# Graylab/DFMDock

Hardware: AMD Instinct MI355X
Metric: docking trajectories/sec (N_res~300+300, 40 steps) (higher is better)
Workload: dtype f16

## Files before the change

### dfmdock_amd/csrc/api_forward.hip

```cpp
#include <cstdio>
#include <cstring>
#include <vector>

#include "dfm_device.h"
#include "dfm_engine.h"

using namespace dfm;

int dfm::begin_call(dfm_complex *cx, int B, const EngineSel &sel, bool l0)
{
    int rc = ensure_workspace(cx, B, sel.bf16, l0);
    if (rc) return rc;
    cx->prof = dfm_profile{};
    cx->ev_used = 0; cx->ev_l0_used = 0;
    cx->fwd_counter = 0;
    if (l0) {
        if (!(sel.bf16 ? cx->l0_valid : cx->l0_valid32)) {
            float bms = 0.f;
            if ((rc = build_l0_table(cx, &bms, !sel.bf16)) != DFM_OK) return rc;
            cx->prof.l0_build_ms = bms;
        }
        HIPCHK(hipMemsetAsync(cx->ws.l0_miss_total, 0, sizeof(unsigned long long), cx->stream));
    }
    return DFM_OK;
// ... 205 lines not shown
        cx->prof.l0_evals += 1; cx->prof.l0_edges += (int64_t)B * N * K;
    }
    return DFM_OK;
}

static int enqueue_messages(const Fwd &f, int l, const float *h, bool lig_only)
{
    EdgeArgs e = layer_edge_args(f, l, lig_only);
    int rc = enqueue_layer_telemetry(f, l, h, e);
    if (rc) return rc;
    rc = (l == 0 && f.o.l0_table) ? enqueue_l0_table(f, e) : enqueue_message_launch(f, e);
    if (rc) return rc;
    if (e.last && f.o.bf16) HIPCHK(launch_coord_bf16(e, f.cx->stream));
    return DFM_OK;
}

static int enqueue_node_model(const Fwd &f, int l, const float *h, float *hn)
{
    dfm_complex *cx = f.cx;
    const FwdOpts &o = f.o;
    Workspace &W = cx->ws;
    hipStream_t s = cx->stream;
    const LayerDev &Lw = cx->m->layers[l];
    const int N = cx->N;
    const bool last = (l == cx->m->hp.depth - 1);
    GemmArgs g = gemm_args(h, H, 2 * H, Lw.W3, 2 * H, Lw.b3, f.M, H, W.u, H);
    g.A1 = W.agg; g.pro = 1; g.a0_period = l == 0 ? N : 0;
    const bool fused_stats = o.bf16 && gemm_rows_per_tile() == 64;
    if (fused_stats) { g.stat_part = W.gn_part; g.rows_per_graph = N; }
    HIPCHK(launch_gemm(o.bf16, g, Lw.W3_hi, Lw.W3_lo, s));
    if (!fused_stats) HIPCHK(launch_gn_stats(W.u, f.B, N, Lw.gn_ms, W.gn_shift, W.gn_den, o.bf16 ? Lw.gn_w : nullptr, o.bf16 ? Lw.gn_b : nullptr, s));
    g = gemm_args(W.u, H, H, Lw.W4, H, Lw.b4, f.M, H, hn, H);
    g.pro = 2; g.gn_shift = W.gn_shift; g.gn_den = W.gn_den; g.gn_w = Lw.gn_w; g.gn_b = Lw.gn_b; g.rows_per_graph = N;
    if (fused_stats) { g.gn_part = W.gn_part; g.gn_ms = Lw.gn_ms; }
    if (o.bf16 && !last && f.tile_tasks) g.zbuf = W.agg;
    g.epi = 1; g.R = h; g.r_period = l == 0 ? N : 0;
    HIPCHK(launch_gemm(o.bf16, g, Lw.W4_hi, Lw.W4_lo, s));
    return DFM_OK;
}

static int enqueue_next_ab(const Fwd &f, int l, const float *h)
{
    dfm_complex *cx = f.cx;
    const FwdOpts &o = f.o;
    Workspace &W = cx->ws;
    const LayerDev &Ln = cx->m->layers[l];
    const float *bias = cx->homomer ? (o.bf16 ? Ln.bias_ab_h_s : Ln.bias_ab_h) : (o.bf16 ? Ln.bias_ab_s : Ln.bias_ab);
    GemmArgs g = gemm_args(h, H, H, Ln.Wab, H, bias, f.M, 2 * H, W.A, H);
    g.epi = 2; g.C2 = o.bf16 ? nullptr : W.Bm; g.C2b = W.Bmb;
    if (o.bf16 && !o.f16) g.Cb = reinterpret_cast<uint16_t *>(W.A);
    HIPCHK(launch_gemm(o.bf16, g, Ln.Wab_hi, Ln.Wab_lo, cx->stream));
    return DFM_OK;
}

static int enqueue_pair_head(const Fwd &f, int q, int mode)
{
    dfm_complex *cx = f.cx;
    const dfm_model *m = cx->m;
    Workspace &W = cx->ws;
    hipStream_t s = cx->stream;
    const int R = cx->R;
    const PairHeadDev &Ph = m->pair[q];
    HIPCHK(project_ab(cx, f.B, Ph.wab, Ph.wab_hi, Ph.wab_lo, f.o.bf16));
    PairArgs a;
    std::memset(&a, 0, sizeof(a));
    a.P = W.A; a.Q = W.Bm; a.ca4 = W.ca4; a.B = f.B; a.R = R; a.L = cx->L; a.w_d = Ph.w_d; a.ln_w = Ph.ln_w; a.ln_b = Ph.ln_b;
    a.w3 = Ph.w3; a.mode = mode; a.cut_off = m->hp.cut_off; a.fpart = W.fpart;
    a.spart = mode == 1 ? W.en_part : W.cpart; a.clash_part = W.clash_part;
    if (f.o.bf16) {
        a.S = W.pair_s; a.Rp = (R + 31) / 32 * 32;
        HIPCHK(launch_pair_head_m(a, s));
        HIPCHK(launch_pair_finish_s(a, 4 * ((R + 63) / 64), m->hp.agg_mean ? 1.0f / (float)R : 1.0f, W.fvec, W.conf, s));
        return DFM_OK;
    }
    HIPCHK(launch_pair_head(a, s));
    return DFM_OK;
}

static int enqueue_pair_heads(const Fwd &f)
{
    dfm_complex *cx = f.cx;
    const dfm_model *m = cx->m;
    Workspace &W = cx->ws;
// ... 13 lines not shown
{
    dfm_complex *cx = f.cx;
    const dfm_model *m = cx->m;
    Workspace &W = cx->ws;
    hipStream_t s = cx->stream;
    GemmArgs g = gemm_args(W.h, H, H, m->heads.en_wa, 2 * H, nullptr, f.M, H, W.A, H);
    HIPCHK(launch_gemm_f32(g, s));
    g.W = m->heads.en_wb; g.C = W.Bm;
    HIPCHK(launch_gemm_f32(g, s));
    HIPCHK(launch_energy_pairs(W.A, W.Bm, W.ca4, f.B, cx->R, cx->L, m->hp.cut_off, &m->heads, 1, W.en_part, W.clash_part, s));
    return DFM_OK;
}

int dfm::enqueue_forward(dfm_complex *cx, int B, const FwdOpts &o)
{
    const dfm_model *m = cx->m;
    Workspace &W = cx->ws;
    hipStream_t s = cx->stream;
    const int depth = m->hp.depth;
    const Fwd f{cx, o, B, B * cx->N, m->hp.family == 1, o.bf16 && edge_msg_tile_tasks(B, cx->N, cx->K)};
    int rc = enqueue_graph(f, cx->fwd_counter++);
    if (rc) return rc;
    const float *h = cx->h0;
    float *hn = W.h, *hspare = W.h2;
    for (int l = 0; l < depth; ++l) {
        const bool last = (l == depth - 1);
        const bool lig_only = last && !f.pair_family && !o.need_node_out;
        if ((rc = enqueue_messages(f, l, h, lig_only)) != DFM_OK) return rc;
        if (lig_only) break;
        if ((rc = enqueue_node_model(f, l, h, hn)) != DFM_OK) return rc;
        { float *done = hn; hn = (l == 0) ? hspare : const_cast<float *>(h); h = done; }
        if (l == 0 && o.h_first_out)
            HIPCHK(hipMemcpyAsync(o.h_first_out, h, (size_t)f.M * H * sizeof(float), hipMemcpyDeviceToDevice, s));
        if (!last && (rc = enqueue_next_ab(f, l + 1, h)) != DFM_OK) return rc;
    }
    if (o.range && (o.need_node_out || f.pair_family)) HIPCHK(launch_absmax(h, (long long)f.M * H, o.range + depth * 8, s));
    if (h != W.h && (o.need_node_out || f.pair_family))
        HIPCHK(hipMemcpyAsync(W.h, h, (size_t)f.M * H * sizeof(float), hipMemcpyDeviceToDevice, s));
    if (f.pair_family) return enqueue_pair_heads(f);
    if (o.want_energy) return enqueue_energy_head(f);
    return DFM_OK;
}

int dfm::finish_profile(dfm_complex *cx)
{
    float ms = 0.f;
    HIPCHK(hipEventElapsedTime(&ms, cx->ev_total[0], cx->ev_total[1]));
    cx->prof.total_ms = ms;
    for (size_t i = 0; i + 1 < cx->ev_used; i += 2) {
        HIPCHK(hipEventElapsedTime(&ms, cx->ev[i], cx->ev[i + 1]));
        cx->prof.edge_kernel_ms += ms;
        if (i / 2 < cx->ev_lig.size() && cx->ev_lig[i / 2]) cx->prof.edge_lig_ms += ms;
    }
    for (size_t i = 0; i + 2 < cx->ev_l0_used; i += 3) {
        HIPCHK(hipEventElapsedTime(&ms, cx->ev_l0[i], cx->ev_l0[i + 1]));
        cx->prof.l0_rows_ms += ms;
        HIPCHK(hipEventElapsedTime(&ms, cx->ev_l0[i + 1], cx->ev_l0[i + 2]));
        cx->prof.l0_gather_ms += ms;
    }
    if (cx->prof.l0_evals > 0 && cx->ws.l0_miss_total) {
        unsigned long long tot = 0;
        HIPCHK(hipMemcpyAsync(&tot, cx->ws.l0_miss_total, sizeof(tot), hipMemcpyDeviceToHost, cx->stream));
        HIPCHK(hipStreamSynchronize(cx->stream));
        cx->prof.l0_miss_rows = (int64_t)tot;
    }
#if !defined(DFM_EDGE_STAMP) && !defined(DFM_EDGE_TRACE)
    if (cx->stamp_dev && cx->ev_used) {
// ... 40 lines not shown
```

### dfmdock_amd/csrc/dfm_internal.h

```cpp
#pragma once

#include <hip/hip_runtime.h>
#include <cstdlib>
#include <stdint.h>

#include <atomic>

#include "../../include/dfmdock_amd.h"
#include "dfm_schedule.h"
#include "dfm_walkgrid.h"

namespace dfm {

constexpr int H = 256;
constexpr int HE = 128;
constexpr int HI = 128;
constexpr int NTAB = 166;
constexpr int KPAD = 64;
constexpr int MAX_NODES = 4096;
constexpr float SILU_S = -1.44269504088896340736f;

__host__ __device__ inline uint32_t pack_code(int d, int om, int th, int ph, int rp)
{
    return (uint32_t)d | ((uint32_t)om << 6) | ((uint32_t)th << 11) | ((uint32_t)ph << 16) | ((uint32_t)rp << 20);
// ... 69 lines not shown
    if (e != hipSuccess) return e;
    if (dev < 0 || dev >= MAX_DEVICES) return hipErrorInvalidDevice;
    if (done[dev].load(std::memory_order_acquire)) return hipSuccess;
    e = hipFuncSetAttribute(fn, hipFuncAttributeMaxDynamicSharedMemorySize, bytes);
    if (e == hipSuccess) done[dev].store(true, std::memory_order_release);
    return e;
}

struct GemmArgs {
    const float *A0;
    const float *A1;
    int lda;
    int K;
    const float *W;
    int ldw;
    const float *bias;
    int M, Nout;
    int pro;
    const float *gn_shift;
    const float *gn_den;
    const float *gn_w, *gn_b;
    int rows_per_graph;
    int epi;
    const float *R;
    float *C;
    int ldc;
    float *C2;
    uint16_t *C2b;
    uint16_t *Cb;
    float *stat_part;
    const float *gn_part, *gn_ms;
    float *zbuf;
    int a0_period, r_period;
};
hipError_t launch_gemm_f32(const GemmArgs &a, hipStream_t s);
hipError_t launch_gemm_split(const GemmArgs &a, const uint16_t *Whi, const uint16_t *Wlo, hipStream_t s);
int gemm_rows_per_tile();

inline unsigned token_lds()
{
    static const unsigned v = [] { const char *e = getenv("DFM_TOKEN_LDS"); return e ? (unsigned)atoi(e) : 64u; }();
    return v;
}

hipError_t launch_prep_pose(const float *rec_pos, const float *lig_cur, int B, int R, int L, int all_atoms, float4 *n4,
                            float4 *ca4, float4 *cb4, hipStream_t s);
hipError_t launch_knn_sample(const float4 *ca4, int B, int N, int knn, int nsamp, uint64_t seed, uint32_t stream_id,
                             int32_t *edges, const uint32_t *ctl, hipStream_t s);
struct L0Classify {
    const uint2 *code0;
    uint32_t *src;
    uint4 *rows;
    uint32_t *counter;
};
hipError_t launch_edge_feat(const float4 *n4, const float4 *ca4, const float4 *cb4, const int32_t *edges, int B,
                            int N, int R, int K, float mask_dist, uint32_t *codes, float *radial, const L0Classify &cls,
                            uint32_t *eval_ctr , hipStream_t s);
hipError_t launch_l0_pairs(const float4 *n4, const float4 *ca4, const float4 *cb4, int R, int L, float mask_dist, uint2 *code0,
                           uint4 *rows, hipStream_t s);

constexpr int TASK_CTR_WGS = 1024;
struct EdgeArgs {
    const float *A;
    const float *Bm;
    const uint16_t *Bmb;
    const uint16_t *Ah;
    int64_t ab_bstride;
    const int32_t *edges;
    const uint32_t *codes;
    const float *radial;
// ... 316 lines not shown
```

### dfmdock_amd/csrc/kernels_dense.hip

```cpp
#include <cstdlib>
#include "dfm_device.h"
#include "dfm_internal.h"

namespace dfm {

typedef float f32x16 __attribute__((ext_vector_type(16)));

constexpr int BM = 128, BN = 128, BK = 16, LDT = BM + 1;

__global__ __launch_bounds__(256) void k_gemm_f32(GemmArgs a)
{
    __shared__ float As[BK * LDT];
    __shared__ float Ws[BK * LDT];
    const int tid = threadIdx.x, lane = tid & 63, wave = tid >> 6;
    const int wm = wave >> 1, wn = wave & 1;
    const int row0 = blockIdx.x * BM, col0 = blockIdx.y * BN;

    f32x16 acc[2][2];
#pragma unroll
    for (int i = 0; i < 2; ++i)
#pragma unroll
        for (int j = 0; j < 2; ++j)
#pragma unroll
            for (int r = 0; r < 16; ++r) acc[i][j][r] = 0.f;

    const int lr = tid >> 2;
    const int lk = (tid & 3) * 4;
    const int halfK = a.K >> 1;

    for (int k0 = 0; k0 < a.K; k0 += BK) {
#pragma unroll
        for (int rr = 0; rr < 2; ++rr) {
            const int r = lr + rr * 64;
            const int grow = row0 + r;
            const int grow_a = a.a0_period ? grow % a.a0_period : grow;
// ... 215 lines not shown
#pragma unroll
        for (int u = 0; u < GN_CH; ++u) {
            const int t = t0 + u;
            if (t < tpt) {
                const double nt = (double)(N - t * 32 < 32 ? N - t * 32 : 32), m = (double)v[u].x, w = nt * m;
                S1 += w; S2 += w * m; SM += (double)v[u].y;
            }
        }
    }
    const double mean = S1 / N;
    const double M2 = SM + (S2 - mean * S1);
    const float sft = (float)mean * mean_scale[c];
    const double dm = mean - (double)sft;
    double var = M2 / N + dm * dm;
    var = var > 0 ? var : 0;
    const float dn = sqrtf((float)var + 1e-5f);
    if (fold_w) {
        const float sc = fold_w[c] / dn;
        o_den = sc;
        o_shift = fold_b[c] - sc * sft;
    } else {
        o_shift = sft;
        o_den = dn;
    }
}

typedef __bf16 bf16x8 __attribute__((ext_vector_type(8)));
union FragB { uint4 u; bf16x8 b; };
constexpr int SK = 32, SLD = 40;

struct GemmSplitArgs {
    GemmArgs g;
    const uint16_t *Whi, *Wlo;
};

__device__ inline uint32_t pack2(__bf16 a, __bf16 b)
{
    union { __bf16 h[2]; uint32_t u; } v;
    v.h[0] = a; v.h[1] = b;
    return v.u;
}

template <int HALF, int NJ, int QT = 0, int RING = QT> __global__ __launch_bounds__(256, RING ? 1 : 3) void k_gemm_split(GemmSplitArgs sa)
{
    static_assert(!QT || NJ == 1, "quarter tiles: one 32-column tile per wave");
    static_assert(!RING || NJ == 1, "the register ring is sized for the 64 x 128 and 64 x 64 shapes");
    static_assert(!QT || RING, "quarter tiles always run the ring");
    constexpr int MI = QT ? 1 : 2;
    constexpr int SM = 64, SN = QT ? 64 : NJ * 128;
    const GemmArgs &a = sa.g;
#ifdef DFM_GEMM_STAMP
    const unsigned long long g_entry = __builtin_amdgcn_s_memtime(), g_rt0 = __builtin_amdgcn_s_memrealtime();
#endif
    constexpr int LDS_BUF = (2 * SM + 2 * SN) * SLD;
    constexpr int LDS_OPER = (RING ? 2 : 1) * LDS_BUF, LDS_EPI = 4 * 32 * 72 * 2;
    constexpr int LDS_U16 = LDS_OPER > LDS_EPI ? LDS_OPER : LDS_EPI;
    __shared__ __attribute__((aligned(16))) uint16_t lds[LDS_U16];
    uint16_t *Ah = lds, *Al = lds + SM * SLD, *Wh = lds + 2 * SM * SLD, *Wl = lds + (2 * SM + SN) * SLD;
    const int tid = threadIdx.x, lane = tid & 63, wave = tid >> 6;
    const int wm = QT ? wave >> 1 : 0, wn = QT ? wave & 1 : wave, l31 = lane & 31;
    __shared__ __attribute__((aligned(16))) float gn_s[2 * H];
    const int vb = blockIdx.x;
    int bx = vb, by = blockIdx.y;
    if (NJ == 2 && gridDim.y == 1 && a.Nout == 2 * SN) {
        const int g16 = bx >> 4, j = bx & 15;
        bx = g16 * 8 + (j & 7); by = j >> 3;
        if (bx * SM >= a.M) return;
    }
    int row0 = bx * SM, row_end = a.M, gn_tb = 0;
    const int col0 = by * SN;
    if (a.stat_part || a.pro == 2) {
        const int tpt = (a.rows_per_graph + SM - 1) / SM, tb = bx / tpt;
        row0 = tb * a.rows_per_graph + (bx - tb * tpt) * SM;
        row_end = (tb + 1) * a.rows_per_graph;
        gn_tb = tb;
    }
    if (a.zbuf) {
        const int zr = tid >> 2;
        if (row0 + zr < row_end) {
            float4 *z = reinterpret_cast<float4 *>(a.zbuf + (size_t)(row0 + zr) * H + col0 + (tid & 3) * (SN / 4));
#pragma unroll
            for (int q = 0; q < SN / 16; ++q) z[q] = make_float4(0.f, 0.f, 0.f, 0.f);
        }
    }
    constexpr int LPR = SN * 4 / 128, NTOUCH = QT ? (SM * LPR + 255) / 256 : 0;
    float touch[NTOUCH + 1];
#pragma unroll
    for (int q = 0; q < NTOUCH; ++q) {
        touch[q] = 0.f;
        const int t = tid + q * 256, row = row0 + t / LPR;
        if (a.epi == 1 && t < SM * LPR && row < row_end) {
            const int rrow = a.r_period ? row % a.r_period : row;
            touch[q] = a.R[(size_t)rrow * a.ldc + col0 + (t % LPR) * 32];
        }
    }
    f32x16 acc[MI][NJ];
#pragma unroll
    for (int i = 0; i < MI; ++i)
#pragma unroll
        for (int j = 0; j < NJ; ++j)
#pragma unroll
            for (int r = 0; r < 16; ++r) acc[i][j][r] = 0.f;

    const int ar = tid >> 2, kg = (tid & 3) * 8;
    const int halfK = a.K >> 1;
    const bool rv0 = row0 + ar < row_end;
    const size_t gr0 = (size_t)(rv0 ? row0 + ar : 0);
    const size_t gr0a = a.a0_period ? gr0 % (size_t)a.a0_period : gr0;

    float4 xa0, xa1;
    uint4 wh0, wh1, wh2, wh3, wl0, wl1, wl2, wl3;
    const int wcol = QT ? (tid & 63) : (NJ == 2 ? tid : (tid & 127));
    const int wkq = QT ? (tid >> 7) * 2 : 0;
    const uint16_t *wsrc = QT ? (((tid >> 6) & 1) ? sa.Wlo : sa.Whi) : ((NJ == 2 || tid < 128) ? sa.Whi : sa.Wlo);
#define GEMM_SPLIT_FETCH(K0)                                                                                          \
    {                                                                                                                 \
        const int k_ = (K0) + kg;                                                                                     \
        const bool second_ = a.pro == 1 && k_ >= halfK;                                                               \
        const float *s0_ = second_ ? a.A1 + (k_ - halfK) + gr0 * a.lda : a.A0 + k_ + gr0a * a.lda;                    \
        xa0 = *reinterpret_cast<const float4 *>(s0_); xa1 = *reinterpret_cast<const float4 *>(s0_ + 4);              \
        const size_t wbase_ = ((size_t)((K0) / SK) * 4 * a.Nout + col0 + wcol) * 8;                                   \
        const size_t wq_ = (size_t)a.Nout * 8;                                                                        \
        const uint16_t *ph_ = wsrc + wbase_ + wkq * wq_, *pl_ = sa.Wlo + wbase_;                                      \
        wh0 = *reinterpret_cast<const uint4 *>(ph_); wh1 = *reinterpret_cast<const uint4 *>(ph_ + wq_);               \
        if constexpr (!QT) {                                                                                          \
            wh2 = *reinterpret_cast<const uint4 *>(ph_ + 2 * wq_); wh3 = *reinterpret_cast<const uint4 *>(ph_ + 3 * wq_); \
        }                                                                                                             \
        if constexpr (NJ == 2) {                                                                                      \
            wl0 = *reinterpret_cast<const uint4 *>(pl_); wl1 = *reinterpret_cast<const uint4 *>(pl_ + wq_);               \
            wl2 = *reinterpret_cast<const uint4 *>(pl_ + 2 * wq_); wl3 = *reinterpret_cast<const uint4 *>(pl_ + 3 * wq_); \
        }                                                                                                             \
    }
    auto stage_row = [&](const float4 &v0, const float4 &v1, bool , int k, int row, int boff = 0) {
        float x[8] = {v0.x, v0.y, v0.z, v0.w, v1.x, v1.y, v1.z, v1.w};
        if (a.pro == 2) {
            const float4 c0 = *reinterpret_cast<const float4 *>(&gn_s[k]), c1 = *reinterpret_cast<const float4 *>(&gn_s[k + 4]);
            const float4 h0 = *reinterpret_cast<const float4 *>(&gn_s[H + k]), h1 = *reinterpret_cast<const float4 *>(&gn_s[H + k + 4]);
            const float cc[8] = {c0.x, c0.y, c0.z, c0.w, c1.x, c1.y, c1.z, c1.w};
            const float hh[8] = {h0.x, h0.y, h0.z, h0.w, h1.x, h1.y, h1.z, h1.w};
#pragma unroll
            for (int e = 0; e < 8; ++e) {
                const float y = fmaf(x[e], cc[e], hh[e]);
                x[e] = y * __builtin_amdgcn_rcpf(1.0f + __expf(-y));
            }
        }
        uint32_t hi[4], lo[4];
#pragma unroll
        for (int e = 0; e < 4; ++e) {
            const float x0 = x[2 * e], x1 = x[2 * e + 1];
            const __bf16 b0 = (__bf16)x0, b1 = (__bf16)x1;
            hi[e] = pack2(b0, b1);
            lo[e] = pack2((__bf16)(x0 - (float)b0), (__bf16)(x1 - (float)b1));
        }
// ... 12 lines not shown
#endif
    float bias_r[NJ];
#pragma unroll
    for (int j = 0; j < NJ; ++j) bias_r[j] = a.bias ? a.bias[col0 + (wn * NJ + j) * 32 + l31] : 0.f;
    constexpr int QD = RING ? 4 : 1, RW = QT ? 2 : 4;
    float4 rxa0[QD], rxa1[QD];
    uint4 rw[QD][RW];
    GEMM_SPLIT_FETCH(0)
#define RING_TAKE(d) { rxa0[d] = xa0; rxa1[d] = xa1; rw[d][0] = wh0; rw[d][1] = wh1; if constexpr (!QT) { rw[d][2] = wh2; rw[d][3] = wh3; } }
#define RING_WSTORE(d, nb) { _Pragma("unroll") for (int q_ = 0; q_ < RW; ++q_) *reinterpret_cast<uint4 *>(&wdst[(nb) + wu + 8 * q_]) = rw[d][q_]; }
    if constexpr (RING) {
        RING_TAKE(0)
#pragma unroll
        for (int d = 1; d < QD; ++d) {
            GEMM_SPLIT_FETCH((d * SK < a.K ? d : 0) * SK)
            RING_TAKE(d)
        }
    }
    if (a.pro == 2) {
        if (a.gn_part) {
            float sc, sh;
            gn_finish_col(a.gn_part, gn_tb, a.rows_per_graph, tid, a.gn_ms, a.gn_w, a.gn_b, sc, sh);
            gn_s[tid] = sc; gn_s[H + tid] = sh;
        } else if (tid < 128) {
            const float *src = (tid < 64 ? a.gn_den : a.gn_shift) + (size_t)gn_tb * H + (tid & 63) * 4;
            *reinterpret_cast<float4 *>(&gn_s[(tid < 64 ? 0 : H) + (tid & 63) * 4]) = *reinterpret_cast<const float4 *>(src);
        }
        __syncthreads();
    }
    auto mfma_stage = [&](int boff = 0) {
#pragma unroll
        for (int ks = 0; ks < SK; ks += 16) {
            const int ko = ks + (lane >> 5) * 8;
            FragB ah[MI], al[MI];
#pragma unroll
            for (int i = 0; i < MI; ++i) {
                const int r = (wm * MI + i) * 32 + l31;
                ah[i].u = *reinterpret_cast<const uint4 *>(&Ah[boff + r * SLD + ko]);
                al[i].u = *reinterpret_cast<const uint4 *>(&Al[boff + r * SLD + ko]);
            }
#pragma unroll
            for (int j = 0; j < NJ; ++j) {
                const int c = (wn * NJ + j) * 32 + l31;
                FragB wh, wl;
                wh.u = *reinterpret_cast<const uint4 *>(&Wh[boff + c * SLD + ko]);
                wl.u = *reinterpret_cast<const uint4 *>(&Wl[boff + c * SLD + ko]);
#pragma unroll
                for (int i = 0; i < MI; ++i) {
                    acc[i][j] = __builtin_amdgcn_mfma_f32_32x32x16_bf16(al[i].b, wh.b, acc[i][j], 0, 0, 0);
                    acc[i][j] = __builtin_amdgcn_mfma_f32_32x32x16_bf16(ah[i].b, wl.b, acc[i][j], 0, 0, 0);
                    acc[i][j] = __builtin_amdgcn_mfma_f32_32x32x16_bf16(ah[i].b, wh.b, acc[i][j], 0, 0, 0);
                }
            }
        }
    };
    if constexpr (RING) {
        const int S = a.K / SK;
        stage_row(rxa0[0], rxa1[0], rv0, kg, ar, 0);
        RING_WSTORE(0, 0)
        {
            GEMM_SPLIT_FETCH((QD < S ? QD : S - 1) * SK)
            RING_TAKE(0)
        }
        __syncthreads();
        GSTAMP(1)
        for (int k0 = 0; k0 < S; k0 += QD) {
#pragma unroll
            for (int d = 0; d < QD; ++d) {
                const int k = k0 + d;
                const int dn = (d + 1) % QD, nb = ((d + 1) & 1) * LDS_BUF;
                const int kn = k + 1 < S ? k + 1 : S - 1, kf = k + 1 + QD < S ? k + 1 + QD : S - 1;
                mfma_stage((d & 1) * LDS_BUF);
                GSTAMP(0)
                stage_row(rxa0[dn], rxa1[dn], rv0, kn * SK + kg, ar, nb);
                RING_WSTORE(dn, nb)
                {
                    GEMM_SPLIT_FETCH(kf * SK)
                    RING_TAKE(dn)
                }
                GSTAMP(1)
                __syncthreads();
                GSTAMP(2)
            }
        }
    } else {
        for (int k0 = 0; k0 < a.K; k0 += SK) {
            if (k0) __syncthreads();
            GSTAMP(0)
            stage_row(xa0, xa1, rv0, k0 + kg, ar);
            *reinterpret_cast<uint4 *>(&wdst[wu]) = wh0; *reinterpret_cast<uint4 *>(&wdst[wu + 8]) = wh1;
            if constexpr (!QT) { *reinterpret_cast<uint4 *>(&wdst[wu + 16]) = wh2; *reinterpret_cast<uint4 *>(&wdst[wu + 24]) = wh3; }
            if constexpr (NJ == 2) {
                *reinterpret_cast<uint4 *>(&Wl[wu]) = wl0; *reinterpret_cast<uint4 *>(&Wl[wu + 8]) = wl1;
                *reinterpret_cast<uint4 *>(&Wl[wu + 16]) = wl2; *reinterpret_cast<uint4 *>(&Wl[wu + 24]) = wl3;
            }
            GSTAMP(1)
            __syncthreads();
            GSTAMP(2)
            if (k0 + SK < a.K) GEMM_SPLIT_FETCH(k0 + SK)
            mfma_stage();
        }
    }
#pragma unroll
    for (int q = 0; q < NTOUCH; ++q) asm volatile("" :: "v"(touch[q]));
    GSTAMP(0)
    __syncthreads();
    constexpr int ELD = 72;
    float *est = reinterpret_cast<float *>(lds) + wave * (32 * ELD);
    const int er = lane >> 4, ec = (lane & 15) * 4;
    float st_s[MI][4], st_q[MI][4], st_p[MI][4], st_n[MI];
#pragma unroll
    for (int i = 0; i < MI; ++i) {
        st_n[i] = 0.f;
#pragma unroll
        for (int e = 0; e < 4; ++e) { st_s[i][e] = 0.f; st_q[i][e] = 0.f; st_p[i][e] = 0.f; }
    }
#pragma unroll
    for (int i = 0; i < MI; ++i)
#pragma unroll
        for (int jp = 0; jp < (NJ + 1) / 2; ++jp) {
            float4 res[8];
            if (a.epi == 1) {
#pragma unroll
                for (int q = 0; q < 8; ++q) {
                    const size_t row = (size_t)row0 + (wm * MI + i) * 32 + q * 4 + er;
                    const size_t rrow = a.r_period ? row % (size_t)a.r_period : row;
                    const int col = col0 + (wn * NJ + jp * 2) * 32 + ec;
                    res[q] = (row < (size_t)row_end && ec < NJ * 32) ? *reinterpret_cast<const float4 *>(a.R + rrow * a.ldc + col) : make_float4(0.f, 0.f, 0.f, 0.f);
                }
            }
#pragma unroll
            for (int jj = 0; jj < (NJ < 2 ? NJ : 2); ++jj) {
                const int j = jp * 2 + jj;
                const float bias = bias_r[j];
#pragma unroll
                for (int r = 0; r < 16; ++r)
                    est[((r & 3) + 8 * (r >> 2) + 4 * (lane >> 5)) * ELD + jj * 32 + l31] = acc[i][j][r] + bias;
            }
            asm volatile("s_waitcnt lgkmcnt(0)" ::: "memory");
            if constexpr (HALF) {
                uint16_t *half_out = col0 < H ? a.Cb : a.C2b;
                const int er8 = lane >> 3, ec8 = (lane & 7) * 8;
#pragma unroll
                for (int q = 0; q < 4; ++q) {
                    const int lr = q * 8 + er8;
                    const float4 v0 = *reinterpret_cast<const float4 *>(est + lr * ELD + ec8);
                    const float4 v1 = *reinterpret_cast<const float4 *>(est + lr * ELD + ec8 + 4);
                    const size_t row = (size_t)row0 + (wm * MI + i) * 32 + lr;
                    const int col = (col0 < H ? col0 : col0 - H) + (wn * NJ + jp * 2) * 32 + ec8;
                    if (row >= (size_t)row_end || ec8 >= NJ * 32) continue;
                    uint4 o;
// ... 18 lines not shown
                        st_q[i][0] += d0 * d0; st_q[i][1] += d1 * d1; st_q[i][2] += d2 * d2; st_q[i][3] += d3 * d3;
                        st_n[i] += 1.f;
                    }
                }
                if (a.epi == 1) {
                    const float4 rr = res[q];
                    *reinterpret_cast<float4 *>(a.C + row * a.ldc + col) = make_float4(rr.x + v.x, rr.y + v.y, rr.z + v.z, rr.w + v.w);
                } else if (a.epi == 2) {
                    if (col0 < H) {
                        if (a.Cb) {
                            uint2 o;
                            o.x = pack_h2_sat(v.x, v.y);
                            o.y = pack_h2_sat(v.z, v.w);
                            *reinterpret_cast<uint2 *>(a.Cb + row * H + col) = o;
                        } else *reinterpret_cast<float4 *>(a.C + row * H + col) = v;
                    } else {
                        if (a.C2) *reinterpret_cast<float4 *>(a.C2 + row * H + (col - H)) = v;
                        if (a.C2b) {
                            uint2 o;
                            o.x = pack_h2_sat(v.x, v.y);
                            o.y = pack_h2_sat(v.z, v.w);
                            *reinterpret_cast<uint2 *>(a.C2b + row * H + (col - H)) = o;
                        }
                    }
                } else {
                    *reinterpret_cast<float4 *>(a.C + row * a.ldc + col) = v;
                }
            }
            }
            asm volatile("s_waitcnt lgkmcnt(0)" ::: "memory");
        }
    if (a.stat_part) {
#pragma clang fp contract(off)
        const int tpt64 = (a.rows_per_graph + 63) / 64, tpt32 = (a.rows_per_graph + 31) / 32;
#pragma unroll
        for (int i = 0; i < MI; ++i) {
            const int sub = (vb % tpt64) * 2 + wm * MI + i;
            float *sp = a.stat_part + ((size_t)(vb / tpt64) * tpt32 + sub) * (H * 2);
            const float inv_n = st_n[i] > 0.f ? 1.0f / st_n[i] : 0.f;
            float nl[2], fl[2];
            {
                float ne = st_n[i];
#pragma unroll
                for (int lv = 0; lv < 2; ++lv) {
                    const float n2 = __shfl_xor(ne, 16 << lv, 64), nt = ne + n2;
                    nl[lv] = ne;
                    fl[lv] = nt > 0.f ? n2 / nt : 0.f;
                    ne = nt;
                }
            }
#pragma unroll
            for (int e = 0; e < 4; ++e) {
                float mean = st_p[i][e] + st_s[i][e] * inv_n, M2 = st_q[i][e] - st_s[i][e] * st_s[i][e] * inv_n;
#pragma unroll
                for (int lv = 0; lv < 2; ++lv) {
                    const float mean2 = __shfl_xor(mean, 16 << lv, 64), M22 = __shfl_xor(M2, 16 << lv, 64);
                    const float d = mean2 - mean, f = fl[lv];
                    mean += d * f;
                    M2 += M22 + d * d * nl[lv] * f;
                }
                if (er == 0 && ec < NJ * 32 && sub < tpt32) {
                    const int c = col0 + wn * (NJ * 32) + ec + e;
                    sp[c * 2] = mean;
                    sp[c * 2 + 1] = M2;
                }
            }
        }
    }
#ifdef DFM_GEMM_STAMP
    GSTAMP(3)
    if (vb == (gridDim.x > 2048 ? 7 * 8 + 1536 : 3) && blockIdx.y == 0 && tid == 0 && a.C) {
        const unsigned long long g_rt1 = __builtin_amdgcn_s_memrealtime();
        printf("gemm stamp K=%d Nout=%d pro=%d epi=%d stats=%d gn=%d: entry->loop %llu  mfma+barrier %llu  fetch-wait+stage %llu  barrier2 %llu  epilogue %llu  total %llu shader cycles in %llu ticks of 100 MHz = %llu MHz\n",
               a.K, a.Nout, a.pro, a.epi, a.stat_part ? 1 : 0, a.gn_part ? 1 : 0, g_first - g_entry, gs[0], gs[1], gs[2], gs[3], gprev - g_entry, g_rt1 - g_rt0,
               (g_rt1 > g_rt0) ? 100ull * (gprev - g_entry) / (g_rt1 - g_rt0) : 0ull);
    }
#endif
}
#undef GEMM_SPLIT_FETCH

int gemm_rows_per_tile() { return 64; }

hipError_t launch_gemm_split(const GemmArgs &a, const uint16_t *Whi, const uint16_t *Wlo, hipStream_t s)
{
    constexpr int SN = 256;
    if (a.K % SK != 0 || a.Nout % SN != 0 || (a.pro == 1 && (a.K / 2) % SK != 0) || a.lda % 4 != 0 || a.ldc % 4 != 0)
        return hipErrorInvalidValue;
    GemmSplitArgs sa;
    sa.g = a; sa.Whi = Whi; sa.Wlo = Wlo;
    if (a.stat_part && (a.Nout != SN || a.rows_per_graph < 1 || a.M % a.rows_per_graph != 0)) return hipErrorInvalidValue;
    if (a.pro == 2 && (a.rows_per_graph < 1 || a.M % a.rows_per_graph != 0)) return hipErrorInvalidValue;
    if (a.zbuf && a.Nout != SN) return hipErrorInvalidValue;
    const int row_tiles = (a.stat_part || a.pro == 2) ? (a.M / a.rows_per_graph) * ((a.rows_per_graph + 63) / 64) : (a.M + 63) / 64;
    static const int narrow_env = [] {
        const char *e = getenv("DFM_GEMM_NARROW_MAXWG");
        return e ? atoi(e) : -1;
    }();
    const int narrow_max = narrow_env >= 0 ? narrow_env : 2 * device_cus();
    const bool narrow = (long long)row_tiles * (a.Nout / SN) < narrow_max;
    const bool half = a.epi == 2 && a.Cb && a.C2b && !a.C2;
    if (narrow) {
        static const int quarter_env = [] {
            const char *e = getenv("DFM_GEMM_QUARTER_MAXWG");
            return e ? atoi(e) : -1;
        }();
        const int quarter_max = quarter_env >= 0 ? quarter_env : device_cus() / 2;
        if ((long long)row_tiles * (a.Nout / 128) < quarter_max && (a.K / 32) % 4 == 0) {
            const dim3 grid(row_tiles, a.Nout / 64);
            if (half) hipLaunchKernelGGL((k_gemm_split<1, 1, 1>), grid, dim3(256), 0, s, sa);
            else hipLaunchKernelGGL((k_gemm_split<0, 1, 1>), grid, dim3(256), 0, s, sa);
            return hipGetLastError();
        }
        const dim3 grid(row_tiles, a.Nout / 128);
        if (half) hipLaunchKernelGGL((k_gemm_split<1, 1>), grid, dim3(256), 0, s, sa);
        else hipLaunchKernelGGL((k_gemm_split<0, 1>), grid, dim3(256), 0, s, sa);
        return hipGetLastError();
    }
    dim3 grid;
    if (a.stat_part || a.pro == 2) grid = dim3(row_tiles, a.Nout / SN);
    else if (a.Nout == 2 * SN) grid = dim3((((a.M + 63) / 64 + 7) / 8) * 16, 1);
    else grid = dim3((a.M + 63) / 64, a.Nout / SN);
    if (half) hipLaunchKernelGGL((k_gemm_split<1, 2>), grid, dim3(256), 0, s, sa);
    else hipLaunchKernelGGL((k_gemm_split<0, 2>), grid, dim3(256), 0, s, sa);
    return hipGetLastError();
}

__global__ __launch_bounds__(256) void k_gn_stats(const float *__restrict__ u, int N, const float *__restrict__ mean_scale,
                                                  float *__restrict__ shift, float *__restrict__ den,
                                                  const float *__restrict__ fold_w, const float *__restrict__ fold_b)
{
    __shared__ double red[16][64];
// ... 13 lines not shown
        __syncthreads();
    };
    double s[4] = {0, 0, 0, 0};
    for (int n = rl; n < N; n += 16) {
        const float4 v = *reinterpret_cast<const float4 *>(U + (size_t)n * H);
        s[0] += v.x; s[1] += v.y; s[2] += v.z; s[3] += v.w;
    }
    reduce_rows(s);
    if (threadIdx.x < 64) sh_shift[threadIdx.x] = (float)(red[0][threadIdx.x] / N) * mean_scale[c0 + threadIdx.x];
    __syncthreads();
    const float4 sft = *reinterpret_cast<const float4 *>(&sh_shift[cq * 4]);
    double v2[4] = {0, 0, 0, 0};
    for (int n = rl; n < N; n += 16) {
        const float4 v = *reinterpret_cast<const float4 *>(U + (size_t)n * H);
        const float o0 = v.x - sft.x, o1 = v.y - sft.y, o2 = v.z - sft.z, o3 = v.w - sft.w;
        v2[0] += (double)o0 * o0; v2[1] += (double)o1 * o1; v2[2] += (double)o2 * o2; v2[3] += (double)o3 * o3;
    }
    reduce_rows(v2);
    if (threadIdx.x < 64) {
        const int c = c0 + threadIdx.x;
        const float var = (float)(red[0][threadIdx.x] / N);
        const float dn = sqrtf(var + 1e-5f), sf = sh_shift[threadIdx.x];
        if (fold_w) {
            const float sc = fold_w[c] / dn;
            den[(size_t)b * H + c] = sc;
            shift[(size_t)b * H + c] = fold_b[c] - sc * sf;
        } else {
            shift[(size_t)b * H + c] = sf;
            den[(size_t)b * H + c] = dn;
        }
    }
}

hipError_t launch_gn_stats(const float *u, int B, int N, const float *mean_scale, float *shift, float *den,
                           const float *fold_w, const float *fold_b, hipStream_t s)
{
    hipLaunchKernelGGL(k_gn_stats, dim3(B, 4), dim3(256), 0, s, u, N, mean_scale, shift, den, fold_w, fold_b);
    return hipGetLastError();
}

}
```

Baseline: 456.4.

## Skip dead GEMM work: lean tail tiles, receptor-only rows, one-time GN finish

Adds a lean mode, on by default, with three parts. In the node-model GEMMs, partial tail tiles with fewer than 32 live rows run a single-row-block variant in which only two waves stage A, so MFMA and loads on padding rows are skipped. In the last layer's A/B projection for ligand-only output, tiles covering only receptor rows in the first half of the columns exit early. GroupNorm statistics are finished once by a small separate kernel instead of redundantly inside every W4 GEMM tile, at the cost of an extra launch. The tile-to-trajectory mapping is also reordered so full tiles come first, which adds complexity in the stat_part indexing.

```diff
diff --git a/dfmdock_amd/csrc/api_forward.hip b/dfmdock_amd/csrc/api_forward.hip
--- a/dfmdock_amd/csrc/api_forward.hip
+++ b/dfmdock_amd/csrc/api_forward.hip
@@ -261,14 +261,16 @@
     if (!fused_stats) HIPCHK(launch_gn_stats(W.u, f.B, N, Lw.gn_ms, W.gn_shift, W.gn_den, o.bf16 ? Lw.gn_w : nullptr, o.bf16 ? Lw.gn_b : nullptr, s));
     g = gemm_args(W.u, H, H, Lw.W4, H, Lw.b4, f.M, H, hn, H);
     g.pro = 2; g.gn_shift = W.gn_shift; g.gn_den = W.gn_den; g.gn_w = Lw.gn_w; g.gn_b = Lw.gn_b; g.rows_per_graph = N;
-    if (fused_stats) { g.gn_part = W.gn_part; g.gn_ms = Lw.gn_ms; }
+    const bool finish_once = fused_stats && gemm_finish_once(f.B, N);
+    if (finish_once) HIPCHK(launch_gn_finish(W.gn_part, f.B, N, Lw.gn_ms, Lw.gn_w, Lw.gn_b, W.gn_den, W.gn_shift, s));
+    else if (fused_stats) { g.gn_part = W.gn_part; g.gn_ms = Lw.gn_ms; }
     if (o.bf16 && !last && f.tile_tasks) g.zbuf = W.agg;
     g.epi = 1; g.R = h; g.r_period = l == 0 ? N : 0;
     HIPCHK(launch_gemm(o.bf16, g, Lw.W4_hi, Lw.W4_lo, s));
     return DFM_OK;
 }
 
-static int enqueue_next_ab(const Fwd &f, int l, const float *h)
+static int enqueue_next_ab(const Fwd &f, int l, const float *h, bool lig_only)
 {
     dfm_complex *cx = f.cx;
     const FwdOpts &o = f.o;
@@ -278,6 +280,7 @@
     GemmArgs g = gemm_args(h, H, H, Ln.Wab, H, bias, f.M, 2 * H, W.A, H);
     g.epi = 2; g.C2 = o.bf16 ? nullptr : W.Bm; g.C2b = W.Bmb;
     if (o.bf16 && !o.f16) g.Cb = reinterpret_cast<uint16_t *>(W.A);
+    if (lig_only && o.bf16 && !o.range && !o.sat) { g.lig_N = cx->N; g.lig_R = cx->R; }
     HIPCHK(launch_gemm(o.bf16, g, Ln.Wab_hi, Ln.Wab_lo, cx->stream));
     return DFM_OK;
 }
@@ -357,7 +360,8 @@
         { float *done = hn; hn = (l == 0) ? hspare : const_cast<float *>(h); h = done; }
         if (l == 0 && o.h_first_out)
             HIPCHK(hipMemcpyAsync(o.h_first_out, h, (size_t)f.M * H * sizeof(float), hipMemcpyDeviceToDevice, s));
-        if (!last && (rc = enqueue_next_ab(f, l + 1, h)) != DFM_OK) return rc;
+        const bool next_lig_only = (l + 1 == depth - 1) && !f.pair_family && !o.need_node_out;
+        if (!last && (rc = enqueue_next_ab(f, l + 1, h, next_lig_only)) != DFM_OK) return rc;
     }
     if (o.range && (o.need_node_out || f.pair_family)) HIPCHK(launch_absmax(h, (long long)f.M * H, o.range + depth * 8, s));
     if (h != W.h && (o.need_node_out || f.pair_family))
diff --git a/dfmdock_amd/csrc/dfm_gemm_map.h b/dfmdock_amd/csrc/dfm_gemm_map.h
--- /dev/null
+++ b/dfmdock_amd/csrc/dfm_gemm_map.h
@@ -0,0 +1,36 @@
+#pragma once
+
+#if defined(__HIPCC__) || defined(__CUDACC__)
+#define DFM_MAP_FN __host__ __device__ inline
+#else
+#define DFM_MAP_FN inline
+#endif
+
+namespace dfm {
+
+struct GemmTile {
+    int traj;
+    int tile;
+};
+
+DFM_MAP_FN GemmTile gemm_aligned_tile(int vb, int rows_per_graph, int M, int lean)
+{
+    const int tpt = (rows_per_graph + 63) / 64, full = rows_per_graph / 64;
+    GemmTile t;
+    if (!lean || full == tpt || full == 0) {
+        t.traj = vb / tpt; t.tile = vb - t.traj * tpt;
+        return t;
+    }
+    const int n_full = (M / rows_per_graph) * full;
+    if (vb < n_full) { t.traj = vb / full; t.tile = vb - t.traj * full; }
+    else { t.traj = vb - n_full; t.tile = full; }
+    return t;
+}
+
+DFM_MAP_FN bool gemm_rows_receptor_only(int row0, int row_end, int N, int R)
+{
+    const int p = row0 % N;
+    return p < R && row_end <= row0 - p + R;
+}
+
+}
diff --git a/dfmdock_amd/csrc/dfm_internal.h b/dfmdock_amd/csrc/dfm_internal.h
--- a/dfmdock_amd/csrc/dfm_internal.h
+++ b/dfmdock_amd/csrc/dfm_internal.h
@@ -125,10 +125,15 @@
     const float *gn_part, *gn_ms;
     float *zbuf;
     int a0_period, r_period;
+    int lig_N, lig_R;
 };
 hipError_t launch_gemm_f32(const GemmArgs &a, hipStream_t s);
 hipError_t launch_gemm_split(const GemmArgs &a, const uint16_t *Whi, const uint16_t *Wlo, hipStream_t s);
 int gemm_rows_per_tile();
+bool gemm_lean();
+bool gemm_finish_once(int B, int N);
+hipError_t launch_gn_finish(const float *part, int B, int N, const float *mean_scale, const float *fold_w, const float *fold_b,
+                            float *den, float *shift, hipStream_t s);
 
 inline unsigned token_lds()
 {
diff --git a/dfmdock_amd/csrc/kernels_dense.hip b/dfmdock_amd/csrc/kernels_dense.hip
--- a/dfmdock_amd/csrc/kernels_dense.hip
+++ b/dfmdock_amd/csrc/kernels_dense.hip
@@ -1,6 +1,8 @@
 #include <cstdlib>
+#include <type_traits>
 #include "dfm_device.h"
 #include "dfm_internal.h"
+#include "dfm_gemm_map.h"
 
 namespace dfm {
 
@@ -282,6 +284,7 @@
 struct GemmSplitArgs {
     GemmArgs g;
     const uint16_t *Whi, *Wlo;
+    int lean;
 };
 
 __device__ inline uint32_t pack2(__bf16 a, __bf16 b)
@@ -291,48 +294,22 @@
     return v.u;
 }
 
-template <int HALF, int NJ, int QT = 0, int RING = QT> __global__ __launch_bounds__(256, RING ? 1 : 3) void k_gemm_split(GemmSplitArgs sa)
-{
-    static_assert(!QT || NJ == 1, "quarter tiles: one 32-column tile per wave");
-    static_assert(!RING || NJ == 1, "the register ring is sized for the 64 x 128 and 64 x 64 shapes");
-    static_assert(!QT || RING, "quarter tiles always run the ring");
-    constexpr int MI = QT ? 1 : 2;
+template <int HALF, int NJ, int QT, int RING, bool DEAD>
+__device__ __forceinline__ void gemm_split_tile(const GemmSplitArgs &sa, uint16_t *lds, float *gn_s, int row0, int row_end, int col0,
+                                                int gn_tb, int tile_in)
+{
+    constexpr int MI = QT ? 1 : 2, ML = DEAD ? 1 : MI;
     constexpr int SM = 64, SN = QT ? 64 : NJ * 128;
+    constexpr int LDS_BUF = (2 * SM + 2 * SN) * SLD;
     const GemmArgs &a = sa.g;
 #ifdef DFM_GEMM_STAMP
     const unsigned long long g_entry = __builtin_amdgcn_s_memtime(), g_rt0 = __builtin_amdgcn_s_memrealtime();
+    const int vb = blockIdx.x;
 #endif
-    constexpr int LDS_BUF = (2 * SM + 2 * SN) * SLD;
-    constexpr int LDS_OPER = (RING ? 2 : 1) * LDS_BUF, LDS_EPI = 4 * 32 * 72 * 2;
-    constexpr int LDS_U16 = LDS_OPER > LDS_EPI ? LDS_OPER : LDS_EPI;
-    __shared__ __attribute__((aligned(16))) uint16_t lds[LDS_U16];
     uint16_t *Ah = lds, *Al = lds + SM * SLD, *Wh = lds + 2 * SM * SLD, *Wl = lds + (2 * SM + SN) * SLD;
     const int tid = threadIdx.x, lane = tid & 63, wave = tid >> 6;
     const int wm = QT ? wave >> 1 : 0, wn = QT ? wave & 1 : wave, l31 = lane & 31;
-    __shared__ __attribute__((aligned(16))) float gn_s[2 * H];
-    const int vb = blockIdx.x;
-    int bx = vb, by = blockIdx.y;
-    if (NJ == 2 && gridDim.y == 1 && a.Nout == 2 * SN) {
-        const int g16 = bx >> 4, j = bx & 15;
-        bx = g16 * 8 + (j & 7); by = j >> 3;
-        if (bx * SM >= a.M) return;
-    }
-    int row0 = bx * SM, row_end = a.M, gn_tb = 0;
-    const int col0 = by * SN;
-    if (a.stat_part || a.pro == 2) {
-        const int tpt = (a.rows_per_graph + SM - 1) / SM, tb = bx / tpt;
-        row0 = tb * a.rows_per_graph + (bx - tb * tpt) * SM;
-        row_end = (tb + 1) * a.rows_per_graph;
-        gn_tb = tb;
-    }
-    if (a.zbuf) {
-        const int zr = tid >> 2;
-        if (row0 + zr < row_end) {
-            float4 *z = reinterpret_cast<float4 *>(a.zbuf + (size_t)(row0 + zr) * H + col0 + (tid & 3) * (SN / 4));
-#pragma unroll
-            for (int q = 0; q < SN / 16; ++q) z[q] = make_float4(0.f, 0.f, 0.f, 0.f);
-        }
-    }
+    const int wave_u = __builtin_amdgcn_readfirstlane(wave);
     constexpr int LPR = SN * 4 / 128, NTOUCH = QT ? (SM * LPR + 255) / 256 : 0;
     float touch[NTOUCH + 1];
 #pragma unroll
@@ -344,9 +321,9 @@
             touch[q] = a.R[(size_t)rrow * a.ldc + col0 + (t % LPR) * 32];
         }
     }
-    f32x16 acc[MI][NJ];
-#pragma unroll
-    for (int i = 0; i < MI; ++i)
+    f32x16 acc[ML][NJ];
+#pragma unroll
+    for (int i = 0; i < ML; ++i)
 #pragma unroll
         for (int j = 0; j < NJ; ++j)
 #pragma unroll
@@ -363,12 +340,16 @@
     const int wcol = QT ? (tid & 63) : (NJ == 2 ? tid : (tid & 127));
     const int wkq = QT ? (tid >> 7) * 2 : 0;
     const uint16_t *wsrc = QT ? (((tid >> 6) & 1) ? sa.Wlo : sa.Whi) : ((NJ == 2 || tid < 128) ? sa.Whi : sa.Wlo);
-#define GEMM_SPLIT_FETCH(K0)                                                                                          \
+#define GEMM_SPLIT_FETCH_A(K0)                                                                                        \
     {                                                                                                                 \
         const int k_ = (K0) + kg;                                                                                     \
         const bool second_ = a.pro == 1 && k_ >= halfK;                                                               \
         const float *s0_ = second_ ? a.A1 + (k_ - halfK) + gr0 * a.lda : a.A0 + k_ + gr0a * a.lda;                    \
         xa0 = *reinterpret_cast<const float4 *>(s0_); xa1 = *reinterpret_cast<const float4 *>(s0_ + 4);              \
+    }
+#define GEMM_SPLIT_FETCH(K0) GEMM_SPLIT_FETCH_A(K0) GEMM_SPLIT_FETCH_W(K0)
+#define GEMM_SPLIT_FETCH_W(K0)                                                                                        \
+    {                                                                                                                 \
         const size_t wbase_ = ((size_t)((K0) / SK) * 4 * a.Nout + col0 + wcol) * 8;                                   \
         const size_t wq_ = (size_t)a.Nout * 8;                                                                        \
         const uint16_t *ph_ = wsrc + wbase_ + wkq * wq_, *pl_ = sa.Wlo + wbase_;                                      \
@@ -447,9 +428,9 @@
 #pragma unroll
         for (int ks = 0; ks < SK; ks += 16) {
             const int ko = ks + (lane >> 5) * 8;
-            FragB ah[MI], al[MI];
-#pragma unroll
-            for (int i = 0; i < MI; ++i) {
+            FragB ah[ML], al[ML];
+#pragma unroll
+            for (int i = 0; i < ML; ++i) {
                 const int r = (wm * MI + i) * 32 + l31;
                 ah[i].u = *reinterpret_cast<const uint4 *>(&Ah[boff + r * SLD + ko]);
                 al[i].u = *reinterpret_cast<const uint4 *>(&Al[boff + r * SLD + ko]);
@@ -461,7 +442,7 @@
                 wh.u = *reinterpret_cast<const uint4 *>(&Wh[boff + c * SLD + ko]);
                 wl.u = *reinterpret_cast<const uint4 *>(&Wl[boff + c * SLD + ko]);
 #pragma unroll
-                for (int i = 0; i < MI; ++i) {
+                for (int i = 0; i < ML; ++i) {
                     acc[i][j] = __builtin_amdgcn_mfma_f32_32x32x16_bf16(al[i].b, wh.b, acc[i][j], 0, 0, 0);
                     acc[i][j] = __builtin_amdgcn_mfma_f32_32x32x16_bf16(ah[i].b, wl.b, acc[i][j], 0, 0, 0);
                     acc[i][j] = __builtin_amdgcn_mfma_f32_32x32x16_bf16(ah[i].b, wh.b, acc[i][j], 0, 0, 0);
@@ -499,10 +480,11 @@
             }
         }
     } else {
+        const bool stager = wave_u < 2;
         for (int k0 = 0; k0 < a.K; k0 += SK) {
             if (k0) __syncthreads();
             GSTAMP(0)
-            stage_row(xa0, xa1, rv0, k0 + kg, ar);
+            if (!DEAD || stager) stage_row(xa0, xa1, rv0, k0 + kg, ar);
             *reinterpret_cast<uint4 *>(&wdst[wu]) = wh0; *reinterpret_cast<uint4 *>(&wdst[wu + 8]) = wh1;
             if constexpr (!QT) { *reinterpret_cast<uint4 *>(&wdst[wu + 16]) = wh2; *reinterpret_cast<uint4 *>(&wdst[wu + 24]) = wh3; }
             if constexpr (NJ == 2) {
@@ -512,7 +494,10 @@
             GSTAMP(1)
             __syncthreads();
             GSTAMP(2)
-            if (k0 + SK < a.K) GEMM_SPLIT_FETCH(k0 + SK)
+            if (k0 + SK < a.K) {
+                if (!DEAD || stager) GEMM_SPLIT_FETCH_A(k0 + SK)
+                GEMM_SPLIT_FETCH_W(k0 + SK)
+            }
             mfma_stage();
         }
     }
@@ -523,15 +508,15 @@
     constexpr int ELD = 72;
     float *est = reinterpret_cast<float *>(lds) + wave * (32 * ELD);
     const int er = lane >> 4, ec = (lane & 15) * 4;
-    float st_s[MI][4], st_q[MI][4], st_p[MI][4], st_n[MI];
-#pragma unroll
-    for (int i = 0; i < MI; ++i) {
+    float st_s[ML][4], st_q[ML][4], st_p[ML][4], st_n[ML];
+#pragma unroll
+    for (int i = 0; i < ML; ++i) {
         st_n[i] = 0.f;
 #pragma unroll
         for (int e = 0; e < 4; ++e) { st_s[i][e] = 0.f; st_q[i][e] = 0.f; st_p[i][e] = 0.f; }
     }
 #pragma unroll
-    for (int i = 0; i < MI; ++i)
+    for (int i = 0; i < ML; ++i)
 #pragma unroll
         for (int jp = 0; jp < (NJ + 1) / 2; ++jp) {
             float4 res[8];
@@ -616,11 +601,11 @@
         }
     if (a.stat_part) {
 #pragma clang fp contract(off)
-        const int tpt64 = (a.rows_per_graph + 63) / 64, tpt32 = (a.rows_per_graph + 31) / 32;
-#pragma unroll
-        for (int i = 0; i < MI; ++i) {
-            const int sub = (vb % tpt64) * 2 + wm * MI + i;
-            float *sp = a.stat_part + ((size_t)(vb / tpt64) * tpt32 + sub) * (H * 2);
+        const int tpt32 = (a.rows_per_graph + 31) / 32;
+#pragma unroll
+        for (int i = 0; i < ML; ++i) {
+            const int sub = tile_in * 2 + wm * MI + i;
+            float *sp = a.stat_part + ((size_t)gn_tb * tpt32 + sub) * (H * 2);
             const float inv_n = st_n[i] > 0.f ? 1.0f / st_n[i] : 0.f;
             float nl[2], fl[2];
             {
@@ -662,8 +647,70 @@
 #endif
 }
 #undef GEMM_SPLIT_FETCH
+#undef GEMM_SPLIT_FETCH_A
+#undef GEMM_SPLIT_FETCH_W
+
+template <int HALF, int NJ, int QT = 0, int RING = QT> __global__ __launch_bounds__(256, RING ? 1 : 3) void k_gemm_split(GemmSplitArgs sa)
+{
+    static_assert(!QT || NJ == 1, "quarter tiles: one 32-column tile per wave");
+    static_assert(!RING || NJ == 1, "the register ring is sized for the 64 x 128 and 64 x 64 shapes");
+    static_assert(!QT || RING, "quarter tiles always run the ring");
+    constexpr int SM = 64, SN = QT ? 64 : NJ * 128;
+    const GemmArgs &a = sa.g;
+    constexpr int LDS_BUF = (2 * SM + 2 * SN) * SLD;
+    constexpr int LDS_OPER = (RING ? 2 : 1) * LDS_BUF, LDS_EPI = 4 * 32 * 72 * 2;
+    constexpr int LDS_U16 = LDS_OPER > LDS_EPI ? LDS_OPER : LDS_EPI;
+    __shared__ __attribute__((aligned(16))) uint16_t lds[LDS_U16];
+    __shared__ __attribute__((aligned(16))) float gn_s[2 * H];
+    const int vb = blockIdx.x;
+    int bx = vb, by = blockIdx.y;
+    if (NJ == 2 && gridDim.y == 1 && a.Nout == 2 * SN) {
+        const int g16 = bx >> 4, j = bx & 15;
+        bx = g16 * 8 + (j & 7); by = j >> 3;
+        if (bx * SM >= a.M) return;
+    }
+    int row0 = bx * SM, row_end = a.M, gn_tb = 0, tile_in = 0;
+    const int col0 = by * SN;
+    if (a.lig_N && col0 < H && gemm_rows_receptor_only(row0, row0 + SM < a.M ? row0 + SM : a.M, a.lig_N, a.lig_R)) return;
+    if (a.stat_part || a.pro == 2) {
+        const GemmTile gt = gemm_aligned_tile(bx, a.rows_per_graph, a.M, NJ == 2 ? sa.lean : 0);
+        row0 = gt.traj * a.rows_per_graph + gt.tile * SM;
+        row_end = (gt.traj + 1) * a.rows_per_graph;
+        gn_tb = gt.traj; tile_in = gt.tile;
+    }
+    const bool dead1 = NJ == 2 && sa.lean && row0 + 32 >= row_end;
+    const int tid = threadIdx.x;
+    if (a.zbuf) {
+        const int zr = tid >> 2;
+        if (row0 + zr < row_end) {
+            float4 *z = reinterpret_cast<float4 *>(a.zbuf + (size_t)(row0 + zr) * H + col0 + (tid & 3) * (SN / 4));
+#pragma unroll
+            for (int q = 0; q < SN / 16; ++q) z[q] = make_float4(0.f, 0.f, 0.f, 0.f);
+        }
+    }
+    if constexpr (NJ == 2 && !HALF) {
+        if (dead1) gemm_split_tile<HALF, NJ, QT, RING, true>(sa, lds, gn_s, row0, row_end, col0, gn_tb, tile_in);
+        else gemm_split_tile<HALF, NJ, QT, RING, false>(sa, lds, gn_s, row0, row_end, col0, gn_tb, tile_in);
+    } else {
+        gemm_split_tile<HALF, NJ, QT, RING, false>(sa, lds, gn_s, row0, row_end, col0, gn_tb, tile_in);
+    }
+}
 
 int gemm_rows_per_tile() { return 64; }
+
+bool gemm_lean()
+{
+    static const int lean_env = [] { const char *e = getenv("DFM_GEMM_LEAN"); return e ? atoi(e) : 1; }();
+    return lean_env != 0;
+}
+static int gemm_narrow_max()
+{
+    static const int narrow_env = [] {
+        const char *e = getenv("DFM_GEMM_NARROW_MAXWG");
+        return e ? atoi(e) : -1;
+    }();
+    return narrow_env >= 0 ? narrow_env : 2 * device_cus();
+}
 
 hipError_t launch_gemm_split(const GemmArgs &a, const uint16_t *Whi, const uint16_t *Wlo, hipStream_t s)
 {
@@ -675,12 +722,12 @@
     if (a.stat_part && (a.Nout != SN || a.rows_per_graph < 1 || a.M % a.rows_per_graph != 0)) return hipErrorInvalidValue;
     if (a.pro == 2 && (a.rows_per_graph < 1 || a.M % a.rows_per_graph != 0)) return hipErrorInvalidValue;
     if (a.zbuf && a.Nout != SN) return hipErrorInvalidValue;
+    if (a.lig_N && (a.epi != 2 || a.stat_part || a.pro == 2 || a.lig_N < 1 || a.lig_R < 0 || a.lig_R > a.lig_N || a.M % a.lig_N != 0))
+        return hipErrorInvalidValue;
+    sa.lean = gemm_lean() ? 1 : 0;
+    if (!sa.lean) sa.g.lig_N = sa.g.lig_R = 0;
     const int row_tiles = (a.stat_part || a.pro == 2) ? (a.M / a.rows_per_graph) * ((a.rows_per_graph + 63) / 64) : (a.M + 63) / 64;
-    static const int narrow_env = [] {
-        const char *e = getenv("DFM_GEMM_NARROW_MAXWG");
-        return e ? atoi(e) : -1;
-    }();
-    const int narrow_max = narrow_env >= 0 ? narrow_env : 2 * device_cus();
+    const int narrow_max = gemm_narrow_max();
     const bool narrow = (long long)row_tiles * (a.Nout / SN) < narrow_max;
     const bool half = a.epi == 2 && a.Cb && a.C2b && !a.C2;
     if (narrow) {
@@ -760,6 +807,30 @@
     }
 }
 
+__global__ __launch_bounds__(256) void k_gn_finish(const float *__restrict__ part, int N, const float *__restrict__ mean_scale,
+                                                   const float *__restrict__ fold_w, const float *__restrict__ fold_b,
+                                                   float *__restrict__ den, float *__restrict__ shift)
+{
+    float sc, sh;
+    gn_finish_col(part, blockIdx.x, N, threadIdx.x, mean_scale, fold_w, fold_b, sc, sh);
+    den[(size_t)blockIdx.x * H + threadIdx.x] = sc;
+    shift[(size_t)blockIdx.x * H + threadIdx.x] = sh;
+}
+
+bool gemm_finish_once(int B, int N)
+{
+    if (!gemm_lean() || B < 1 || N < 1) return false;
+    return (long long)B * ((N + 63) / 64) >= gemm_narrow_max();
+}
+
+hipError_t launch_gn_finish(const float *part, int B, int N, const float *mean_scale, const float *fold_w, const float *fold_b,
+                            float *den, float *shift, hipStream_t s)
+{
+    if (B < 1 || N < 1 || !fold_w || !fold_b) return hipErrorInvalidValue;
+    hipLaunchKernelGGL(k_gn_finish, dim3(B), dim3(256), token_lds(), s, part, N, mean_scale, fold_w, fold_b, den, shift);
+    return hipGetLastError();
+}
+
 hipError_t launch_gn_stats(const float *u, int B, int N, const float *mean_scale, float *shift, float *den,
                            const float *fold_w, const float *fold_b, hipStream_t s)
 {
```

After: 456.4, median of 2. Within noise of the previous version (-0.0%).
